# yzang2019/tendermint-fork

Hardware: AMD Instinct MI355X
Metric: ed25519 verifies/sec at 1/8 MI355X (higher is better)
Workload: dtype u32 (GF(2^255-19) radix 2^25.5 limbs, int64 accumulate); 1 GPU; C2: raw batch of 1048576 ed25519 signatures per GPU; signatures_per_gpu=1048576, key_cache=False, parallelism=shard-per-gpu x1

## Files before the change

### include/tmed25519.h

```cpp
#ifndef TMED25519_H
#define TMED25519_H

#include <stddef.h>
#include <stdint.h>

#ifdef __cplusplus
extern "C" {
#endif

#define TMED_OK 0
#define TMED_EINVAL (-1)
#define TMED_ENODEV (-2)
#define TMED_EHIP (-3)
#define TMED_ENOMEM (-4)
#define TMED_ENOKEYSET (-5)
#define TMED_EINTERNAL (-6)

typedef struct tmed_ctx tmed_ctx;

int tmed_device_count(void);

int tmed_init(int device, tmed_ctx **out);
void tmed_destroy(tmed_ctx *ctx);
const char *tmed_strerror(int code);

int tmed_verify_batch(tmed_ctx *ctx, const uint8_t *pubkeys, const uint8_t *sigs, const uint32_t *sig_lens,
                      const uint8_t *msgs, const uint32_t *msg_off, size_t n, uint8_t *out_valid);

int tmed_verify_batch_device(tmed_ctx *ctx, const uint8_t *d_pubkeys, const uint8_t *d_sigs,
                             const uint8_t *d_msgs, const uint32_t *d_msg_off, size_t n, uint8_t *d_out_valid,
                             void *stream);

int tmed_sign_batch(tmed_ctx *ctx, const uint8_t *seeds, const uint8_t *msgs, const uint32_t *msg_off, size_t n,
                    uint8_t *sigs_out, uint8_t *pubkeys_out);
int tmed_sign_batch_device(tmed_ctx *ctx, const uint8_t *d_seeds, const uint8_t *d_msgs, const uint32_t *d_msg_off,
                           size_t n, uint8_t *d_sigs_out, uint8_t *d_pubkeys_out, void *stream);

int tmed_window_stats(tmed_ctx *ctx, uint32_t lane_hist[65], uint32_t wave_hist[65]);

int tmed_b_window_bits(const tmed_ctx *ctx);
int tmed_keyset_b_window_bits(const tmed_ctx *ctx);
int tmed_keyset_a_window_bits(tmed_ctx *ctx, uint64_t handle);
int tmed_keyset_comb_entry(tmed_ctx *ctx, uint64_t handle, uint32_t key, int radix_bits, uint32_t window, uint32_t j,
                           int32_t out[30]);

float tmed_last_kernel_ms(tmed_ctx *ctx);

int tmed_set_kernel_timing(tmed_ctx *ctx, int on);
int tmed_kernel_times(tmed_ctx *ctx, float ms[3], int launches[3]);



int tmed_keyset_load(tmed_ctx *ctx, const uint8_t *pubkeys, size_t n, uint64_t *handle);
int tmed_keyset_free(tmed_ctx *ctx, uint64_t handle);
int tmed_keyset_extend(tmed_ctx *ctx, uint64_t handle, const uint8_t *pubkeys, size_t n, uint32_t *first_index);
int tmed_verify_batch_keyset(tmed_ctx *ctx, uint64_t handle, const uint32_t *val_idx, const uint8_t *sigs,
                             const uint32_t *sig_lens, const uint8_t *msgs, const uint32_t *msg_off, size_t n,
                             uint8_t *out_valid);
int tmed_verify_batch_keyset_device(tmed_ctx *ctx, uint64_t handle, const uint32_t *d_val_idx, const uint8_t *d_sigs,
                                    const uint8_t *d_msgs, const uint32_t *d_msg_off, size_t n, uint8_t *d_out_valid,
                                    void *stream);


int tmed_verify_batch_zip215(tmed_ctx *ctx, const uint8_t *pubkeys, const uint8_t *sigs, const uint32_t *sig_lens,
// ... 287 lines not shown
```

### tendermint-fork_amd/csrc/ctx.h

```cpp
#pragma once
#include <hip/hip_runtime.h>

#include <mutex>
#include <unordered_map>
#include <vector>

#include "../../include/tmed25519.h"
#include "kernels.h"
#include "keycache.h"

struct tmed_ctx;
struct BsStream;

namespace tmed {

struct DevBuf {
  void *p = nullptr;
  size_t cap = 0;
  hipError_t ensure(size_t bytes) {
    if (bytes <= cap) return hipSuccess;
    if (p) (void)hipFree(p);
    p = nullptr;
    cap = 0;
    size_t want = bytes + bytes / 4 + 256;
// ... 161 lines not shown
  int device = 0;
  hipStream_t stream = nullptr;
  hipStream_t copy_stream = nullptr;
  hipEvent_t ev0 = nullptr, ev1 = nullptr;
  float last_ms = 0.f;
  float last_copy_ms = 0.f, last_copy_gap_ms = 0.f;
  hipEvent_t trace_t0 = nullptr;
  float last_at[4] = {0, 0, 0, 0};
  std::mutex mu;
  int4 *d_bcomb = nullptr;
  int4 *d_b16 = nullptr;
  int4 *d_bcomb16 = nullptr;
  int4 *d_b26 = nullptr;
  int4 *d_b24 = nullptr;
  bool b24_tried = false;
  bool b24_on = true;
  bool acomb_on = true;
  int test_fail_ks_alloc = 0;
  int4 *d_slab = nullptr;
  int4 *d_prep = nullptr;
  int4 *d_fin = nullptr;
  int4 *d_fin_pre = nullptr;
  uint32_t slab_slots = 0;
  uint32_t chunk = 0;
  int main_waves = 6;
  uint32_t lat_max = 24576;
  int4 *d_glat = nullptr;
  uint32_t glat_max = 24576;
  bool timing = false;
  uint32_t last_hs_count = 0;
  tmed::KernelTimer timer;
  tmed::DevBuf d_a, d_b, d_msg, d_off, d_out, d_c;
  tmed::HostBuf h_a, h_b, h_msg, h_off, h_out, h_c;
  tmed::VoteSlot vslot[3];
  BsStream *bs = nullptr;
  tmed::Lane lane1;
  tmed::DevBuf d_merkle_lv, d_merkle_tab;
  std::vector<uint64_t> merkle_off;
  tmed::DevBuf d_proof_off, d_proof_out, d_proof_in;
  tmed::HostBuf h_csig;
  tmed::DevBuf d_csig;
  tmed::HostBuf h_hdr;
  tmed::DevBuf d_hdr;
  tmed::HostBuf h_med;
  tmed::DevBuf d_med;
  tmed::DevBuf d_korder;
// ... 19 lines not shown
  hipError_t e = hipSuccess;
  if (s == c->stream) {
    if (c->scratch_foreign) e = hipStreamWaitEvent(s, c->scratch_ev, 0);
  } else {
    if (!c->scratch_foreign) e = hipEventRecord(c->scratch_ev, c->stream);
    if (e == hipSuccess) e = hipStreamWaitEvent(s, c->scratch_ev, 0);
  }
  return e;
}
inline uint32_t last_chunk_count(uint32_t n, uint32_t chunk) {
  if (n == 0) return 0;
  const uint32_t m = n - (n - 1) / kFinCap * kFinCap;
  return m - (m - 1) / chunk * chunk;
}
inline bool generic_uses_glat(const tmed_ctx *c, uint32_t n) { return n <= c->glat_max; }
inline hipError_t generic_verify(tmed_ctx *c, const uint8_t *pub, const uint8_t *sig, const uint8_t *msgs,
                                 const uint32_t *off, uint32_t n, uint8_t *out, hipStream_t s, bool msg_slots,
                                 KernelTimer *timer, const VoteAsm *va = nullptr) {
  if (generic_uses_glat(c, n)) {
    c->last_hs_count = 0;
    return launch_verify_glat(pub, sig, msgs, off, n, out, c->d_bcomb16, c->d_glat, s, msg_slots, timer, va);
  }
  if (va) return hipErrorInvalidValue;
  hipError_t e = launch_verify(pub, sig, msgs, off, n, out, c->d_slab, c->slab_slots, BTabs{c->d_b16, c->d_bcomb16, c->d_b26},
                               c->d_prep, c->d_fin, c->d_fin_pre, s, c->chunk, c->main_waves, msg_slots, timer);
  c->last_hs_count = (e != hipSuccess || c->main_waves == 5) ? 0 : last_chunk_count(n, c->chunk);
  return e;
}
inline hipError_t scratch_release(tmed_ctx *c, hipStream_t s) {
  c->scratch_foreign = s != c->stream;
  return c->scratch_foreign ? hipEventRecord(c->scratch_ev, s) : hipSuccess;
}
}
```

### tendermint-fork_amd/csrc/kernels.h

```cpp
#pragma once
#include <hip/hip_runtime.h>
#include <stddef.h>
#include <stdint.h>

#include "ge25519.h"
#include "signbytes.h"

namespace tmed {

struct KernelTimer {
  static constexpr int kMax = 160;
  hipEvent_t ev[kMax];
  int kind[kMax];
  int n = 0;
  void mark(hipStream_t s, int k) {
    if (n < kMax) { kind[n] = k; (void)hipEventRecord(ev[n++], s); }
  }
};

constexpr uint32_t kThreadsPerBlock = 256;
constexpr uint32_t kSlabSlotBytes = 8 * 128;
constexpr uint32_t kSlabJointSlotBytes = 12 * 128;
inline size_t slab_bytes(uint32_t slots) { return (size_t)slots * kSlabJointSlotBytes; }

constexpr uint32_t kFinCap = 1u << 20;
constexpr int kFinInt4 = 8;
constexpr uint32_t kFinGroupMax = 16;
constexpr uint32_t kFinPreStride = kFinCap + 64;
constexpr size_t kFinBytes = (size_t)kFinCap * kFinInt4 * 16;
constexpr size_t kFinPreBytes = (size_t)kFinPreStride * 3 * 16;

struct BTabs {
  const int4 *b16;
  const int4 *comb16;
  const int4 *b26 = nullptr;
};
constexpr uint32_t kB26Entries = (1u << 25) + 1;
constexpr size_t kB26Bytes = 2 * (size_t)kB26Entries * 128;
hipError_t launch_build_b26(const int4 *comb16, int4 *tab, hipStream_t stream);
constexpr int kB24Windows = 11;
constexpr uint32_t kB24Entries = (1u << 23) + 1;
constexpr size_t kB24Bytes = (size_t)kB24Windows * kB24Entries * 128;
hipError_t launch_build_b24(const int4 *comb16, int4 *tab, hipStream_t stream);
constexpr uint32_t kB16Entries = 32769;
constexpr size_t kB16Bytes = (size_t)kB16Entries * 128;
hipError_t launch_build_b16(int4 *tab, hipStream_t stream);
constexpr size_t kBComb16Bytes = 16 * kB16Bytes;
void host_bcomb16_bases(int32_t out[16 * 40]);
hipError_t launch_build_bcomb16(const int32_t *d_bases, int4 *comb, hipStream_t stream);

hipError_t launch_verify(const uint8_t *pub, const uint8_t *sig, const uint8_t *msgs, const uint32_t *off,
                         uint32_t n, uint8_t *out, int4 *slab, uint32_t slab_stride, BTabs btab,
                         int4 *prep, int4 *fin, int4 *fin_pre, hipStream_t stream, uint32_t chunk = 0,
                         int main_waves = 6, bool msg_slots = false, KernelTimer *timer = nullptr,
                         bool zip215 = false);

hipError_t launch_verify_prep(const uint8_t *pub, const uint8_t *sig, const uint8_t *msgs, const uint32_t *off,
                              bool msg_slots, uint32_t base, uint32_t count, int4 *prep, uint32_t stride,
                              hipStream_t stream);
constexpr uint32_t kZipMax = 1u << 20;

hipError_t launch_sign(const uint8_t *seeds, const uint8_t *msgs, const uint32_t *off, uint32_t n, uint8_t *sig_out,
                       uint8_t *pub_out, const int4 *bcomb, hipStream_t stream);

constexpr uint32_t kPrepSlotBytes = 416;
constexpr uint32_t kPrepTailBytes = 256;

constexpr int kCombWindows = 32;
constexpr int kCombEntries = 129;
constexpr int kCombEntryInt4 = 8;
constexpr size_t kCombBytesPerKey = (size_t)kCombWindows * kCombEntries * kCombEntryInt4 * 16;
constexpr int kKeyChunkBits = 9;
constexpr uint32_t kKeyChunkKeys = 1u << kKeyChunkBits;
constexpr uint32_t kKeyChunksMax = (1u << 24) >> kKeyChunkBits;

// ... 63 lines not shown
```

### tendermint-fork_amd/csrc/kernels.hip

```cpp
#include "kernels.h"
#include "verify_core.h"
#include "verify_hs.h"
#include "kernel_util.h"
#include "rows.h"
#include "votes_dev.h"

namespace tmed {

__device__ int4 kIdentityRow[8] = {{1, 0, 0, 0}, {0, 0, 0, 0}, {1, 0, 0, 0}, {0, 0, 0, 0},
                                          {1, 0, 0, 0}, {0, 0, 0, 0}, {0, 0, 0, 0}, {0, 0, 0, 0}};

__device__ __forceinline__ void slab_st(int4 *p, int4 v) { *p = v; }
__device__ __forceinline__ int4 slab_ld(const int4 *p) { return *p; }

template <int ROWS>
struct SlabTabN {
  int4 *base;
  uint32_t slot;

  __device__ __forceinline__ const int4 *row(int j) const {
    return j == 0 ? kIdentityRow : base + ((size_t)slot * ROWS + (j - 1)) * 8;
  }

  __device__ __forceinline__ void store(int j, const ge_cached &c) const {
    if (j == 0) return;
    int4 *r = base + ((size_t)slot * ROWS + (j - 1)) * 8;
// ... 33 lines not shown

template <int BITS>
struct BPf {
  static constexpr int kBits = BITS;
  const int4 *tab;
  int4 *buf;
  uint32_t lane;
  __device__ __forceinline__ void prefetch(int j) const {
    __builtin_amdgcn_s_waitcnt(0xc07f);
#pragma unroll
    for (int q = 0; q < 8; q++)
      __builtin_amdgcn_global_load_lds((global_void *)(tab + (size_t)j * 8 + q), (lds_void *)(buf + q * 64), 16, 0, 0);
  }
  __device__ __forceinline__ void take(ge_niels &e) const { niels_load(e, buf + lane, 64); }
};

constexpr uint32_t kHsBlock = kThreadsPerBlock;

constexpr int kPrepWaves = 3;
__global__ __launch_bounds__(kHsBlock, kPrepWaves) void verify_prep_kernel(
    const uint8_t *__restrict__ pub, const uint8_t *__restrict__ sig, MsgSrc ms, uint32_t base, uint32_t count,
    int4 *__restrict__ prep, uint32_t stride, uint32_t *__restrict__ place) {
  const uint32_t slot = blockIdx.x * blockDim.x + threadIdx.x;
  if (place && slot == 0) place[0] = place[1] = 0;
  if (slot >= count) return;
  const uint32_t i = base + slot;
  uint32_t pw[8];
  bool sok;
  {
    uint32_t sw[16], k[8], h[16];
    load_row_words(pw, pub + 32 * (size_t)i, 2);
    load_row_words(sw, sig + 64 * (size_t)i, 4);
    const uint8_t *m;
    uint32_t mlen;
    ms.get(i, m, mlen);
    sok = (sw[15] & 0xE0000000u) == 0 && sc_is_canonical(sw + 8);
    sha512_stream(h, sw, pw, 64, m, mlen);
    sc_reduce512(k, h);
#pragma unroll
    for (int q = 0; q < 2; q++)
      prep[(size_t)q * stride + slot] = make_int4((int)k[4 * q], (int)k[4 * q + 1], (int)k[4 * q + 2], (int)k[4 * q + 3]);
#pragma unroll
    for (int q = 0; q < 2; q++) {
      const uint32_t *S = sw + 8 + 4 * q;
      prep[(size_t)(2 + q) * stride + slot] = sok ? make_int4((int)S[0], (int)S[1], (int)S[2], (int)S[3])
                                                  : make_int4(0, 0, 0, 0);
    }
// ... 113 lines not shown
  const int leader = __builtin_ctzll(act);
  fs = (uint32_t)__shfl((int)fs, leader);
  fl = (uint32_t)__shfl((int)fl, leader);
  const uint32_t pos = front ? fs + (uint32_t)__builtin_popcountll(sm & below)
                             : count - 1u - (fl + (uint32_t)__builtin_popcountll(act & ~sm & below));
#pragma unroll
  for (int q = 0; q < kPrepHsInt4; q++)
    prep2[(size_t)q * stride + pos] = make_int4(w[4 * q], w[4 * q + 1], w[4 * q + 2], w[4 * q + 3]);
}

struct HsDigitsDev {
  const int4 *p2;
  uint32_t stride, slot;
  bool active;
  __device__ __forceinline__ uint32_t word(int w) const {
    return active ? reinterpret_cast<const uint32_t *>(p2 + (size_t)(w >> 2) * stride + slot)[w & 3] : 0x88888888u;
  }
  __device__ __forceinline__ uint32_t cword(int w) const { return word(w); }
  __device__ __forceinline__ uint32_t dword(int w) const { return w < 5 ? word(8 + w) : 0x88888888u; }
};

constexpr int kHsWaves = 2;
template <int BB>
__global__ __launch_bounds__(kHsBlock, kHsWaves) void verify_main_hs_kernel(
    uint32_t base, uint32_t count, const int4 *__restrict__ prep, const int4 *__restrict__ prep2, uint32_t stride,
    int4 *__restrict__ slab, const int4 *__restrict__ btab, uint8_t *__restrict__ out, int zip215) {
  __shared__ int4 sbl[kHsBlock / 64][8 * 64];
  __shared__ int4 sbh[kHsBlock / 64][8 * 64];
  const uint32_t slot = blockIdx.x * blockDim.x + threadIdx.x;
  const bool active = slot < count;
  int32_t w[64];
#pragma unroll
  for (int q = 3; q < kPrepHsInt4; q++) {
    const int4 v = active ? prep2[(size_t)q * stride + slot] : make_int4(0, 0, 0, 0);
    w[4 * q] = v.x; w[4 * q + 1] = v.y; w[4 * q + 2] = v.z; w[4 * q + 3] = v.w;
  }
  uint32_t er[8];
#pragma unroll
  for (int j = 0; j < 8; j++) er[j] = (uint32_t)w[13 + j];
  if (BB == 16) {
    uint32_t e[8];
#pragma unroll
    for (int j = 0; j < 8; j++) e[j] = er[j];
    sc_recode_b<16>(er, e);
  }
  fe Rx, Ry;
#pragma unroll
  for (int j = 0; j < 10; j++) { Rx.v[j] = w[21 + j]; Ry.v[j] = w[31 + j]; }
  ge_p3 A;
#pragma unroll
  for (int j = 0; j < 10; j++) { A.X.v[j] = w[44 + j]; A.Y.v[j] = w[54 + j]; }
  if (!active) { fe_1(A.Y); fe_1(Ry); }
  fe_1(A.Z);
  fe_mul(A.T, A.X, A.Y);
  const int flags = w[41];
  int W = active ? (flags >> 8) : 29;
#pragma unroll
  for (int o = 32; o > 0; o >>= 1) {
    const int x = __shfl_xor(W, o);
    W = x > W ? x : W;
  }
  W = __builtin_amdgcn_readfirstlane(W);
  if (W < 29) W = 29;
  if (W > 64) W = 64;
  const uint32_t lane = threadIdx.x & 63u, wv = threadIdx.x >> 6;
  const HsDigitsDev ds{prep2, stride, slot, active};
  SlabTabJ tj{slab, slot};
  const size_t hi = BB == 26 ? (size_t)kB26Entries * kCombEntryInt4 : (size_t)8 * kB16Entries * kCombEntryInt4;
  BPf<BB> bl{btab, sbl[wv], lane};
  BPf<BB> bh{btab + hi, sbh[wv], lane};
  const bool id = verify_main_hsj(ds, (flags & 2) != 0, er, W, A, Rx, Ry, tj, bl, bh, zip215 != 0);
  if (active) out[base + (uint32_t)w[42]] = ((flags & 1) && id) ? 1 : 0;
}

__global__ __launch_bounds__(kThreadsPerBlock) void window_stats_kernel(const int4 *__restrict__ prep2, uint32_t stride,
                                                                       uint32_t count, uint32_t *__restrict__ lane_hist,
                                                                       uint32_t *__restrict__ wave_hist) {
  __shared__ uint32_t lh[65], wh[65];
  for (uint32_t b = threadIdx.x; b < 65; b += blockDim.x) lh[b] = wh[b] = 0;
  __syncthreads();
  const uint32_t slot = blockIdx.x * blockDim.x + threadIdx.x;
  const bool active = slot < count;
  int W = active ? (prep2[(size_t)10 * stride + slot].y >> 8) : 0;
  if (W < 0 || W > 64) W = 64;
  if (active) atomicAdd(&lh[W], 1u);
  int m = W;
#pragma unroll
  for (int o = 32; o > 0; o >>= 1) {
    const int x = __shfl_xor(m, o);
    m = x > m ? x : m;
  }
  if ((threadIdx.x & 63u) == 0 && slot < count) atomicAdd(&wh[m], 1u);
  __syncthreads();
  for (uint32_t b = threadIdx.x; b < 65; b += blockDim.x) {
    if (lh[b]) atomicAdd(&lane_hist[b], lh[b]);
// ... 105 lines not shown
__global__ __launch_bounds__(kThreadsPerBlock) void verify_finish_kernel(
    const int4 *__restrict__ fin, int4 *__restrict__ pre, const uint8_t *__restrict__ sig, uint8_t *__restrict__ out,
    uint32_t fin_base, uint32_t L, uint32_t m, const uint32_t *__restrict__ perm) {
  const uint32_t lane = blockIdx.x * blockDim.x + threadIdx.x;
  if (lane >= L) return;
  FinDev a{fin, pre, sig, out, fin_base, lane, L, m, perm};
  finish_group(a);
}

hipError_t launch_finish(const int4 *fin, int4 *pre, const uint8_t *sig, uint8_t *out, uint32_t fin_base, uint32_t m,
                         hipStream_t stream, const uint32_t *perm = nullptr) {
  if (m == 0) return hipSuccess;
  constexpr uint32_t kLanes = 65536;
  uint32_t G = (m + kLanes - 1) / kLanes;
  if (G < 1) G = 1;
  if (G > kFinGroupMax) G = kFinGroupMax;
  const uint32_t L = (m + G - 1) / G;
  hipLaunchKernelGGL(verify_finish_kernel, dim3((L + kThreadsPerBlock - 1) / kThreadsPerBlock),
                     dim3(kThreadsPerBlock), 0, stream, fin, pre, sig, out, fin_base, L, m, perm);
  return hipGetLastError();
}

hipError_t launch_verify(const uint8_t *pub, const uint8_t *sig, const uint8_t *msgs, const uint32_t *off,
                         uint32_t n, uint8_t *out, int4 *slab, uint32_t slab_stride, BTabs btab,
                         int4 *prep, int4 *fin, int4 *fin_pre, hipStream_t stream, uint32_t chunk, int main_waves,
                         bool msg_slots, KernelTimer *timer, bool zip215) {
  const MsgSrc ms{msgs, off, msg_slots};
  if (chunk == 0 || chunk > slab_stride) chunk = slab_stride;
  if (chunk % kThreadsPerBlock != 0 || slab_stride % kThreadsPerBlock != 0) return hipErrorInvalidValue;
  const bool hs = main_waves != 5 || zip215;
  uint32_t *place = reinterpret_cast<uint32_t *>(reinterpret_cast<char *>(prep) + (size_t)slab_stride * kPrepSlotBytes);
  if (timer) timer->mark(stream, -1);
  for (uint32_t fbase = 0; fbase < n; fbase += kFinCap) {
    const uint32_t m = (n - fbase) < kFinCap ? (n - fbase) : kFinCap;
    for (uint32_t base = fbase; base < fbase + m; base += chunk) {
      const uint32_t count = (fbase + m - base) < chunk ? (fbase + m - base) : chunk;
      const uint32_t blocks = (count + kThreadsPerBlock - 1) / kThreadsPerBlock;
      const uint32_t hblocks = (count + kHsBlock - 1) / kHsBlock;

      hipLaunchKernelGGL(verify_prep_kernel, dim3(hblocks), dim3(kHsBlock), 0, stream, pub, sig, ms, base,
                         count, prep, slab_stride, hs ? place : nullptr);
      if (timer) timer->mark(stream, 0);
      if (hs) {
        int4 *prep2 = prep + (size_t)kPrepInt4 * slab_stride;
        hipLaunchKernelGGL(verify_prep_r_kernel, dim3(hblocks), dim3(kHsBlock), 0, stream, sig, base, count,
                           prep, prep2, slab_stride, place, zip215 ? 1 : 0);
        if (timer) timer->mark(stream, 0);
        if (btab.b26)
          hipLaunchKernelGGL(verify_main_hs_kernel<26>, dim3(hblocks), dim3(kHsBlock), 0, stream, base, count,
                             prep, prep2, slab_stride, slab, btab.b26, out, zip215 ? 1 : 0);
        else
          hipLaunchKernelGGL(verify_main_hs_kernel<16>, dim3(hblocks), dim3(kHsBlock), 0, stream, base, count,
                             prep, prep2, slab_stride, slab, btab.comb16, out, zip215 ? 1 : 0);
      } else {
        hipLaunchKernelGGL(verify_main_kernel, dim3(blocks), dim3(kThreadsPerBlock), 0, stream, base, count, prep,
                           slab_stride, slab, btab.b16, fin, fbase, out);
      }
      if (timer) timer->mark(stream, 1);
      hipError_t e = hipGetLastError();
      if (e != hipSuccess) return e;
    }
    hipError_t e = hs ? hipSuccess : launch_finish(fin, fin_pre, sig, out, fbase, m, stream);
    if (timer) timer->mark(stream, 2);
    if (e != hipSuccess) return e;
  }
  return hipSuccess;
}

hipError_t launch_verify_prep(const uint8_t *pub, const uint8_t *sig, const uint8_t *msgs, const uint32_t *off,
                              bool msg_slots, uint32_t base, uint32_t count, int4 *prep, uint32_t stride,
                              hipStream_t stream) {
  if (count == 0) return hipSuccess;
  if (count > stride) return hipErrorInvalidValue;
  const MsgSrc ms{msgs, off, msg_slots};
  hipLaunchKernelGGL(verify_prep_kernel, dim3((count + kHsBlock - 1) / kHsBlock),
                     dim3(kHsBlock), 0, stream, pub, sig, ms, base, count, prep, stride, nullptr);
// ... 576 lines not shown
```

### tendermint-fork_amd/csrc/tmed_capi.hip

```cpp
#include <hip/hip_runtime.h>
#include <stdlib.h>
#include <string.h>

#include <algorithm>
#include <map>
#include <mutex>
#include <new>
#include <string>

#include "../../include/tmed25519.h"
#include "kernels.h"

#include "ctx.h"
#include "median_host.h"

using namespace tmed;

extern "C" {

int tmed_device_count(void) {
  int n = 0;
  if (hipGetDeviceCount(&n) != hipSuccess) return 0;
  return n;
}
// ... 97 lines not shown
  if (hipSetDevice(device) != hipSuccess) return TMED_EHIP;
  tmed_ctx *c = new tmed_ctx();
  c->device = device;
  hipError_t e = hipStreamCreateWithFlags(&c->stream, hipStreamNonBlocking);
  if (e == hipSuccess) e = hipStreamCreateWithFlags(&c->copy_stream, hipStreamNonBlocking);
  if (e == hipSuccess) e = hipEventCreate(&c->ev0);
  if (e == hipSuccess) e = hipEventCreate(&c->ev1);
  if (e == hipSuccess) e = hipEventCreateWithFlags(&c->scratch_ev, hipEventDisableTiming);
  auto round_up = [](uint32_t v) {
    if (v < kThreadsPerBlock) v = kThreadsPerBlock;
    if (v > (1u << 24)) v = 1u << 24;
    return (v + kThreadsPerBlock - 1) / kThreadsPerBlock * kThreadsPerBlock;
  };
  c->slab_slots = 4096 * kThreadsPerBlock;
  c->chunk = c->slab_slots;
  if (const char *v = getenv("TMED_SLAB_SLOTS")) c->slab_slots = round_up((uint32_t)strtoul(v, nullptr, 10));
  c->chunk = c->slab_slots;
  if (const char *v = getenv("TMED_CHUNK")) c->chunk = std::min(c->slab_slots, round_up((uint32_t)strtoul(v, nullptr, 10)));
  if (const char *v = getenv("TMED_MAIN_WAVES")) c->main_waves = atoi(v) == 5 ? 5 : 6;
  if (const char *v = getenv("TMED_LAT_MAX")) c->lat_max = (uint32_t)strtoul(v, nullptr, 10);
  if (c->lat_max > kLatMax) c->lat_max = kLatMax;
  if (const char *v = getenv("TMED_GLAT_MAX")) c->glat_max = (uint32_t)strtoul(v, nullptr, 10);
  if (c->glat_max > kGLatMax) c->glat_max = kGLatMax;
  if (e == hipSuccess)
    e = hipMalloc((void **)&c->d_slab, slab_bytes(c->slab_slots));
  if (e == hipSuccess) e = hipMalloc((void **)&c->d_prep, (size_t)c->slab_slots * kPrepSlotBytes + kPrepTailBytes);
  if (e == hipSuccess) e = hipMalloc((void **)&c->d_fin, kFinBytes);
  if (e == hipSuccess) e = hipMalloc((void **)&c->d_fin_pre, kFinPreBytes);
  if (e == hipSuccess) e = hipMalloc((void **)&c->d_glat, kGLatHandBytes);
  uint8_t *d_bpub = nullptr, *d_bok = nullptr;
  const uint8_t benc[32] = {0x58, 0x66, 0x66, 0x66, 0x66, 0x66, 0x66, 0x66, 0x66, 0x66, 0x66,
                            0x66, 0x66, 0x66, 0x66, 0x66, 0x66, 0x66, 0x66, 0x66, 0x66, 0x66,
                            0x66, 0x66, 0x66, 0x66, 0x66, 0x66, 0x66, 0x66, 0x66, 0x66};
  if (e == hipSuccess) e = hipMalloc((void **)&c->d_b16, kB16Bytes);
  if (e == hipSuccess) e = launch_build_b16(c->d_b16, c->stream);
  if (e == hipSuccess) e = hipMalloc((void **)&c->d_bcomb16, kBComb16Bytes);
  {
    static int32_t bases[16 * 40];
    static std::once_flag bases_once;
    std::call_once(bases_once, [] { host_bcomb16_bases(bases); });
    int32_t *d_bases = nullptr;
    if (e == hipSuccess) e = hipMalloc((void **)&d_bases, sizeof(bases));
    if (e == hipSuccess) e = hipMemcpy(d_bases, bases, sizeof(bases), hipMemcpyHostToDevice);
    if (e == hipSuccess) e = launch_build_bcomb16(d_bases, c->d_bcomb16, c->stream);
    if (e == hipSuccess) e = hipStreamSynchronize(c->stream);
    if (d_bases) (void)hipFree(d_bases);
  }
  if (e == hipSuccess && !env_off("TMED_B26")) c->d_b26 = bshare_acquire(0, device, c->d_bcomb16, c->stream);
  c->b24_on = !env_off("TMED_B24");
  c->acomb_on = !env_off("TMED_KS_ACOMB");
  if (const char *v = getenv("TMED_TEST_FAIL_KS_ALLOC")) c->test_fail_ks_alloc = atoi(v);
  c->kc_on = !env_off("TMED_KEYCACHE");
  if (const char *v = getenv("TMED_KEYCACHE_GB")) c->kc_budget = (size_t)strtoull(v, nullptr, 10) << 30;
  if (e == hipSuccess) e = hipMalloc((void **)&c->d_bcomb, kCombBytesPerKey);
  if (e == hipSuccess) e = hipMalloc((void **)&d_bpub, 32);
  if (e == hipSuccess) e = hipMalloc((void **)&d_bok, 1);
  if (e == hipSuccess) e = hipMemcpy(d_bpub, benc, 32, hipMemcpyHostToDevice);
  int rc = map_err(e);
  if (rc == TMED_OK) rc = build_comb(c, d_bpub, 1, 0, d_bok, c->d_bcomb);
  if (d_bpub) (void)hipFree(d_bpub);
  if (d_bok) (void)hipFree(d_bok);
  if (rc != TMED_OK) {
    tmed_destroy(c);
    return rc;
  }
  *out = c;
  return TMED_OK;
}

void tmed_destroy(tmed_ctx *c) {
  if (!c) return;
// ... 143 lines not shown
    if (!g_pinned.erase((uintptr_t)p)) return TMED_EINVAL;
  }
  return hipHostFree(p) == hipSuccess ? TMED_OK : TMED_EHIP;
}

int tmed_host_register(void *p, size_t bytes) {
  if (!p || bytes == 0) return TMED_EINVAL;
  if (hipHostRegister(p, bytes, hipHostRegisterDefault) != hipSuccess) return TMED_EHIP;
  std::lock_guard<std::mutex> lk(g_pin_mu);
  g_pinned[(uintptr_t)p] = (uintptr_t)p + bytes;
  return TMED_OK;
}

int tmed_host_unregister(void *p) {
  {
    std::lock_guard<std::mutex> lk(g_pin_mu);
    if (!p || !g_pinned.erase((uintptr_t)p)) return TMED_EINVAL;
  }
  return hipHostUnregister(p) == hipSuccess ? TMED_OK : TMED_EHIP;
}

int tmed_b_window_bits(const tmed_ctx *c) { return c && c->d_b26 ? 26 : 16; }
int tmed_keyset_b_window_bits(const tmed_ctx *c) { return c && c->d_b24 ? 24 : 16; }
int tmed_keyset_a_window_bits(tmed_ctx *c, uint64_t handle) {
  if (!c) return -1;
  std::lock_guard<std::mutex> lk(c->mu);
  const Keyset *k = find_keyset(c, handle);
  if (!k) return -1;
  return !k->comba.empty() && k->comba_n == k->n && c->d_b24 ? kCombABits : 8;
}

int tmed_keyset_comb_entry(tmed_ctx *c, uint64_t handle, uint32_t key, int radix_bits, uint32_t window, uint32_t j,
                           int32_t out[30]) {
  if (!c || !out) return TMED_EINVAL;
  std::lock_guard<std::mutex> lk(c->mu);
  const Keyset *k = find_keyset(c, handle);
  if (!k || key >= k->n) return TMED_EINVAL;
  const int4 *src;
  if (radix_bits == 8) {
    if (window >= (uint32_t)kCombWindows || j >= kCombEntries) return TMED_EINVAL;
    src = k->comb_row(key, (size_t)window * kCombEntries + j);
  } else if (radix_bits == kCombABits) {
    if (k->comba.empty() || key >= k->comba_n || window >= (uint32_t)kCombAWindows) return TMED_EINVAL;
    if (j >= (window + 1 == (uint32_t)kCombAWindows ? kCombATopEntries : kCombAEntries)) return TMED_EINVAL;
    src = k->comba_row_of(key, comba_row((int)window, j));
  } else {
// ... 154 lines not shown
```

### tendermint-fork_amd/csrc/zip215.hip

```cpp
#include <hip/hip_runtime.h>
#include <string.h>
#include <sys/random.h>

#include <stdio.h>
#include <stdlib.h>

#include <vector>

#include "ctx.h"
#include "kernel_util.h"
#include "verify_core.h"
#include "verify_hs.h"
#include "quad.h"

namespace tmed {

constexpr int kZipWin = 16;
constexpr int kZipZWin = 8;
constexpr uint32_t kZipRow = 8;
constexpr uint32_t kZipItemsMax = 16385;
__host__ __device__ __forceinline__ int zip_glog(int w) { return w < 8 ? 1 : (w < 15 ? 2 : 0); }
__host__ __device__ __forceinline__ uint32_t zip_groups(int w) { return w < 8 ? 16385u : (w < 15 ? 8193u : 4098u); }
__host__ __device__ __forceinline__ uint32_t zip_h(int w) { return w == 15 ? 2u : 1u; }
__host__ __device__ __forceinline__ uint32_t zip_level_items(int w, int level) {
// ... 729 lines not shown
  if (e != hipSuccess) return map_err(e);
  memset(g_zip_stats, 0, sizeof g_zip_stats);
  const uint32_t chunk = std::min<uint32_t>(kZipMax, c->slab_slots);
  for (uint32_t base = 0; base < n; base += chunk) {
    const uint32_t N = n - base < chunk ? n - base : chunk;
    uint8_t seed[32];
    if (g_zip_fixed) memcpy(seed, g_zip_seed, 32);
    else if (getrandom(seed, 32, 0) != 32) return TMED_EHIP;
    e = hipMemcpyAsync(z.seed, seed, 32, hipMemcpyHostToDevice, s);
    if (e != hipSuccess) return map_err(e);
    g_zip_stats[0]++;
    constexpr uint32_t kZipSinglyMin = 1u << 14;
    if (N >= kZipSinglyMin && c->zip_count_pending) {
      e = hipEventSynchronize(c->zip_ev);
      if (e != hipSuccess) return map_err(e);
      c->zip_count_pending = false;
      c->zip_dense = *static_cast<const uint32_t *>(c->h_zip.p) != 0;
    }
    if (c->zip_dense && N >= kZipSinglyMin) {
      g_zip_stats[2]++;
      g_zip_stats[3] += N;
      const uint8_t *gm = msg_slots ? msgs + (size_t)base * kVoteSlot : msgs;
      e = launch_verify(pub + 32 * (size_t)base, sig + 64 * (size_t)base, gm, off + base, N, out + base, c->d_slab,
                        c->slab_slots, BTabs{c->d_b16, c->d_bcomb16, c->d_b26}, c->d_prep, c->d_fin, c->d_fin_pre, s,
                        c->chunk, 6, msg_slots, nullptr, true);
      if (e == hipSuccess && !c->zip_ev) e = hipEventCreateWithFlags(&c->zip_ev, hipEventDisableTiming);
      if (e == hipSuccess) e = c->h_zip.ensure(4);
      if (e == hipSuccess) e = hipMemsetAsync(z.flag, 0, 4, s);
      if (e == hipSuccess)
        hipLaunchKernelGGL(zip_count_fail_kernel, dim3((N + 4095) / 4096), dim3(256), 0, s, out + base, N, z.flag);
      if (e == hipSuccess) e = hipGetLastError();
      if (e == hipSuccess) e = hipMemcpyAsync(c->h_zip.p, z.flag, 4, hipMemcpyDeviceToHost, s);
      if (e == hipSuccess) e = hipEventRecord(c->zip_ev, s);
      if (e != hipSuccess) return map_err(e);
      c->zip_count_pending = true;
      continue;
    }
    const uint32_t blocks = (N + kThreadsPerBlock - 1) / kThreadsPerBlock;
    e = launch_verify_prep(pub, sig, msgs, off, msg_slots, base, N, c->d_prep, c->slab_slots, s);
    if (e != hipSuccess) return map_err(e);
    hipLaunchKernelGGL(zip_prep_r_kernel, dim3(blocks), dim3(kThreadsPerBlock), 0, s, sig, base, N, c->d_prep,
                       c->slab_slots, z.seed, (uint64_t)base, z.pts, z.dig, z.cs, kZipMax, out);
    constexpr uint32_t kZipMinGroup = 1u << 14;
    std::vector<std::pair<uint32_t, uint32_t>> level{{0u, N}}, single;
    while (!level.empty()) {
      std::vector<std::pair<uint32_t, uint32_t>> failed;
      for (auto &g : level) {
// ... 5 lines not shown
        g_zip_stats[1]++;
        if (!ok) failed.push_back(g);
      }
      const bool dense = level.size() >= 2 && failed.size() * 2 > level.size();
      std::vector<std::pair<uint32_t, uint32_t>> next;
      for (auto &g : failed) {
        if (!dense && g.second >= 2 * kZipMinGroup) {
          const uint32_t h = g.second / 2;
          next.push_back({g.first, h});
          next.push_back({g.first + h, g.second - h});
        } else {
          single.push_back(g);
        }
      }
      level.swap(next);
    }
    if (N >= kZipSinglyMin) c->zip_dense = !single.empty();
    for (auto &g : single) {
      g_zip_stats[2]++;
      g_zip_stats[3] += g.second;
      const uint32_t lo = base + g.first;
      const uint8_t *gm = msg_slots ? msgs + (size_t)lo * kVoteSlot : msgs;
      e = launch_verify(pub + 32 * (size_t)lo, sig + 64 * (size_t)lo, gm, off + lo, g.second, out + lo, c->d_slab,
                        c->slab_slots, BTabs{c->d_b16, c->d_bcomb16, c->d_b26}, c->d_prep, c->d_fin, c->d_fin_pre, s, c->chunk,
                        6, msg_slots, nullptr, true);
      if (e != hipSuccess) return map_err(e);
    }
  }
  c->last_hs_count = 0;
  return TMED_OK;
}

}

extern "C" {

int tmed_zip215_set_seed(const uint8_t *seed32) {
  const char *t = getenv("TMED_ZIP215_TEST_SEED");
  if (seed32 && !(t && t[0] == '1')) return TMED_EINVAL;
  if (seed32) {
    memcpy(g_zip_seed, seed32, 32);
    g_zip_fixed = true;
  } else {
    g_zip_fixed = false;
  }
  return TMED_OK;
}
// ... 62 lines not shown
```

### tendermint-fork_amd/tmed/_native.py

```python
from __future__ import annotations

import ctypes
import os

PKG_ROOT = os.path.dirname(os.path.dirname(os.path.abspath(__file__)))
LIB_PATH = os.environ.get("TMED_LIB") or os.path.join(PKG_ROOT, "lib", "libtmed25519_hip.so")

TMED_OK = 0
TMED_EINVAL = -1
TMED_ENODEV = -2
TMED_EHIP = -3
TMED_ENOMEM = -4
TMED_ENOKEYSET = -5
TMED_EINTERNAL = -6

_lib = None


class TmedError(RuntimeError):
    def __init__(self, code: int, what: str = ""):
        self.code = code
        msg = lib().tmed_strerror(code).decode() if _lib is not None else str(code)
        super().__init__("%s: %s (code %d)" % (what or "tmed", msg, code))

# ... 39 lines not shown
    l.tmed_keycache_stats.argtypes = [P, P]
    l.tmed_keycache_wait.restype = I
    l.tmed_keycache_wait.argtypes = [P]
    l.tmed_keycache_flush.restype = I
    l.tmed_keycache_flush.argtypes = [P]
    l.tmed_keycache_warm.restype = I
    l.tmed_keycache_warm.argtypes = [P, P]
    l.tmed_verify_batch_keyset.restype = I
    l.tmed_verify_batch_keyset.argtypes = [P, ctypes.c_uint64, P, P, P, P, P, SZ, P]
    l.tmed_verify_batch_keyset_device.restype = I
    l.tmed_verify_batch_keyset_device.argtypes = [P, ctypes.c_uint64, P, P, P, P, SZ, P, P]
    l.tmed_set_kernel_timing.restype = I
    l.tmed_set_kernel_timing.argtypes = [P, I]
    l.tmed_kernel_times.restype = I
    l.tmed_kernel_times.argtypes = [P, ctypes.POINTER(ctypes.c_float), ctypes.POINTER(ctypes.c_int)]
    l.tmed_last_kernel_ms.restype = ctypes.c_float
    l.tmed_last_kernel_ms.argtypes = [P]
    l.tmed_window_stats.restype = I
    l.tmed_window_stats.argtypes = [P, P, P]
    l.tmed_b_window_bits.restype = I
    l.tmed_b_window_bits.argtypes = [P]
    l.tmed_keyset_b_window_bits.restype = I
    l.tmed_keyset_b_window_bits.argtypes = [P]
    l.tmed_keyset_a_window_bits.restype = I
    l.tmed_keyset_a_window_bits.argtypes = [P, ctypes.c_uint64]
    l.tmed_keyset_comb_entry.restype = I
    l.tmed_keyset_comb_entry.argtypes = [P, ctypes.c_uint64, ctypes.c_uint32, ctypes.c_int, ctypes.c_uint32,
                                         ctypes.c_uint32, P]
    l.tmed_host_alloc.restype = I
    l.tmed_host_alloc.argtypes = [SZ, ctypes.POINTER(ctypes.c_void_p)]
    l.tmed_host_free.restype = I
    l.tmed_host_free.argtypes = [P]
    l.tmed_host_register.restype = I
    l.tmed_host_register.argtypes = [P, SZ]
    l.tmed_host_unregister.restype = I
    l.tmed_host_unregister.argtypes = [P]
    l.tmed_verify_batch_zip215.argtypes = [P, P, P, P, P, P, SZ, P]
    l.tmed_verify_batch_zip215_device.argtypes = [P, P, P, P, P, SZ, P, P]
    l.tmed_zip215_set_seed.argtypes = [P]
    l.tmed_zip215_stats.argtypes = [P]
    l.tmed_test_pool_jitter.restype = None
    l.tmed_test_pool_jitter.argtypes = [I]
    l.tmed_test_stream_delay.restype = None
    l.tmed_test_stream_delay.argtypes = [I]
    l.tmed_test_joint_rows.restype = I
    l.tmed_test_joint_rows.argtypes = [P, P, P, P, SZ, P]
    l.tmed_debug_zero_bits.restype = I
    l.tmed_debug_zero_bits.argtypes = [P, SZ, ctypes.POINTER(SZ)]
    _lib = l
    return l


EXPORTED_SYMBOLS = [
    "tmed_device_count", "tmed_init", "tmed_destroy", "tmed_strerror",
    "tmed_verify_batch", "tmed_verify_batch_device",
    "tmed_sign_batch", "tmed_sign_batch_device", "tmed_last_kernel_ms",
    "tmed_vote_sign_bytes", "tmed_valu_peak", "tmed_verify_commits", "tmed_verify_commits_with",
    "tmed_test_pool_jitter", "tmed_test_stream_delay", "tmed_test_joint_rows", "tmed_debug_zero_bits",
    "tmed_keyset_load", "tmed_keyset_free", "tmed_keyset_extend", "tmed_verify_batch_keyset",
    "tmed_keycache_config", "tmed_keycache_stats", "tmed_keycache_flush", "tmed_keycache_warm", "tmed_keycache_wait", "tmed_verify_batch_keyset_device",
    "tmed_set_kernel_timing", "tmed_kernel_times", "tmed_blocksync_verify", "tmed_blocksync_submit", "tmed_blocksync_wait",
    "tmed_merkle_roots", "tmed_valset_hashes", "tmed_header_hashes", "tmed_partset_roots",
    "tmed_commit_hashes", "tmed_txs_hashes",
    "tmed_merkle_proofs", "tmed_partset_proofs", "tmed_txs_proofs", "tmed_merkle_proofs_verify",
    "tmed_light_verify", "tmed_light_verify_with",
    "tmed_median_times", "tmed_median_times_host",
    "tmed_verify_commits_multi", "tmed_blocksync_verify_multi", "tmed_window_stats", "tmed_b_window_bits", "tmed_keyset_b_window_bits", "tmed_keyset_a_window_bits", "tmed_keyset_comb_entry", "tmed_seam_phase_us",
    "tmed_verify_batch_zip215", "tmed_verify_batch_zip215_device", "tmed_zip215_set_seed", "tmed_zip215_stats",
    "tmed_host_alloc", "tmed_host_free", "tmed_host_register", "tmed_host_unregister",
]
```

### tendermint-fork_amd/tmed/engine.py

```python
from __future__ import annotations

import ctypes
from typing import Sequence

import numpy as np

from ._native import TMED_OK, TmedError, lib


def _p(a: np.ndarray):
    return a.ctypes.data_as(ctypes.c_void_p)


def pack_messages(msgs: Sequence[bytes]):
    lens = np.fromiter((len(m) for m in msgs), dtype=np.int64, count=len(msgs))
    off = np.zeros(len(msgs) + 1, dtype=np.int64)
    np.cumsum(lens, out=off[1:])
    if off[-1] >= 2**32:
        raise ValueError("message batch exceeds 4 GiB")
    flat = np.frombuffer(b"".join(msgs), dtype=np.uint8) if off[-1] else np.zeros(1, np.uint8)
    return flat, off.astype(np.uint32)


class PinnedBuffer:
# ... 224 lines not shown

    def set_kernel_timing(self, on: bool) -> None:
        rc = lib().tmed_set_kernel_timing(self._h, 1 if on else 0)
        if rc != TMED_OK:
            raise TmedError(rc, "tmed_set_kernel_timing")

    def kernel_times(self):
        ms, n = (ctypes.c_float * 3)(), (ctypes.c_int * 3)()
        rc = lib().tmed_kernel_times(self._h, ms, n)
        if rc != TMED_OK:
            raise TmedError(rc, "tmed_kernel_times")
        return list(ms), list(n)

    def window_stats(self):
        lh, wh = np.zeros(65, np.uint32), np.zeros(65, np.uint32)
        rc = lib().tmed_window_stats(self._h, _p(lh), _p(wh))
        if rc != TMED_OK:
            raise TmedError(rc, "tmed_window_stats")
        return lh, wh

    def b_window_bits(self) -> int:
        return int(lib().tmed_b_window_bits(self._h))

    def keyset_b_window_bits(self) -> int:
        return int(lib().tmed_keyset_b_window_bits(self._h))

    def keyset_a_window_bits(self, handle: int) -> int:
        return int(lib().tmed_keyset_a_window_bits(self._h, handle))

    def keyset_comb_entry(self, handle: int, key: int, radix_bits: int, window: int, j: int) -> np.ndarray:
        out = np.zeros(30, np.int32)
        rc = lib().tmed_keyset_comb_entry(self._h, handle, key, radix_bits, window, j, out.ctypes.data)
        if rc != 0:
            raise TmedError(rc, "tmed_keyset_comb_entry")
        return out

    def last_kernel_ms(self) -> float:
        return float(lib().tmed_last_kernel_ms(self._h))
```

Measured before the change: 107.4 million verifies/s.

## Make HS main verify kernel persistent with per-wave atomic group claiming

The main HS verify kernel becomes a persistent grid, sized to the resident block count from the occupancy API. Each wave atomically claims 64-signature groups until the work runs out. The per-lane slab scratch is now indexed by resident thread slot rather than signature slot, so the slab allocation shrinks to resident lanes only. This is meant to reduce tail imbalance from variable window counts and to shrink the slab's memory footprint, which may improve cache locality. It adds one atomic per group and depends on the occupancy query being accurate.

```diff
diff --git a/include/tmed25519.h b/include/tmed25519.h
--- a/include/tmed25519.h
+++ b/include/tmed25519.h
@@ -40,6 +40,7 @@
 
 int tmed_b_window_bits(const tmed_ctx *ctx);
 int tmed_keyset_b_window_bits(const tmed_ctx *ctx);
+int tmed_main_resident_lanes(const tmed_ctx *ctx);
 int tmed_keyset_a_window_bits(tmed_ctx *ctx, uint64_t handle);
 int tmed_keyset_comb_entry(tmed_ctx *ctx, uint64_t handle, uint32_t key, int radix_bits, uint32_t window, uint32_t j,
                            int32_t out[30]);
diff --git a/tendermint-fork_amd/csrc/ctx.h b/tendermint-fork_amd/csrc/ctx.h
--- a/tendermint-fork_amd/csrc/ctx.h
+++ b/tendermint-fork_amd/csrc/ctx.h
@@ -207,6 +207,7 @@
   int4 *d_fin = nullptr;
   int4 *d_fin_pre = nullptr;
   uint32_t slab_slots = 0;
+  uint32_t hs_blocks = 0;
   uint32_t chunk = 0;
   int main_waves = 6;
   uint32_t lat_max = 24576;
@@ -272,7 +273,8 @@
     return launch_verify_glat(pub, sig, msgs, off, n, out, c->d_bcomb16, c->d_glat, s, msg_slots, timer, va);
   }
   if (va) return hipErrorInvalidValue;
-  hipError_t e = launch_verify(pub, sig, msgs, off, n, out, c->d_slab, c->slab_slots, BTabs{c->d_b16, c->d_bcomb16, c->d_b26},
+  hipError_t e = launch_verify(pub, sig, msgs, off, n, out, c->d_slab, c->slab_slots, c->hs_blocks,
+                               BTabs{c->d_b16, c->d_bcomb16, c->d_b26},
                                c->d_prep, c->d_fin, c->d_fin_pre, s, c->chunk, c->main_waves, msg_slots, timer);
   c->last_hs_count = (e != hipSuccess || c->main_waves == 5) ? 0 : last_chunk_count(n, c->chunk);
   return e;
diff --git a/tendermint-fork_amd/csrc/kernels.h b/tendermint-fork_amd/csrc/kernels.h
--- a/tendermint-fork_amd/csrc/kernels.h
+++ b/tendermint-fork_amd/csrc/kernels.h
@@ -21,7 +21,12 @@
 constexpr uint32_t kThreadsPerBlock = 256;
 constexpr uint32_t kSlabSlotBytes = 8 * 128;
 constexpr uint32_t kSlabJointSlotBytes = 12 * 128;
-inline size_t slab_bytes(uint32_t slots) { return (size_t)slots * kSlabJointSlotBytes; }
+inline size_t slab_hs_bytes(uint32_t hs_blocks) { return (size_t)hs_blocks * kThreadsPerBlock * kSlabJointSlotBytes; }
+inline size_t slab_bytes(uint32_t slots, uint32_t hs_blocks, int main_waves) {
+  const size_t hs = slab_hs_bytes(hs_blocks), full = (size_t)slots * kSlabSlotBytes;
+  return main_waves == 5 && full > hs ? full : hs;
+}
+hipError_t main_hs_resident_blocks(int device, bool b26, uint32_t *blocks);
 
 constexpr uint32_t kFinCap = 1u << 20;
 constexpr int kFinInt4 = 8;
@@ -50,7 +55,7 @@
 hipError_t launch_build_bcomb16(const int32_t *d_bases, int4 *comb, hipStream_t stream);
 
 hipError_t launch_verify(const uint8_t *pub, const uint8_t *sig, const uint8_t *msgs, const uint32_t *off,
-                         uint32_t n, uint8_t *out, int4 *slab, uint32_t slab_stride, BTabs btab,
+                         uint32_t n, uint8_t *out, int4 *slab, uint32_t slab_stride, uint32_t hs_blocks, BTabs btab,
                          int4 *prep, int4 *fin, int4 *fin_pre, hipStream_t stream, uint32_t chunk = 0,
                          int main_waves = 6, bool msg_slots = false, KernelTimer *timer = nullptr,
                          bool zip215 = false);
diff --git a/tendermint-fork_amd/csrc/kernels.hip b/tendermint-fork_amd/csrc/kernels.hip
--- a/tendermint-fork_amd/csrc/kernels.hip
+++ b/tendermint-fork_amd/csrc/kernels.hip
@@ -2,6 +2,7 @@
 #include "verify_core.h"
 #include "verify_hs.h"
 #include "kernel_util.h"
+#include "main_claim.h"
 #include "rows.h"
 #include "votes_dev.h"
 
@@ -81,7 +82,7 @@
     const uint8_t *__restrict__ pub, const uint8_t *__restrict__ sig, MsgSrc ms, uint32_t base, uint32_t count,
     int4 *__restrict__ prep, uint32_t stride, uint32_t *__restrict__ place) {
   const uint32_t slot = blockIdx.x * blockDim.x + threadIdx.x;
-  if (place && slot == 0) place[0] = place[1] = 0;
+  if (place && slot == 0) place[0] = place[1] = place[2] = 0;
   if (slot >= count) return;
   const uint32_t i = base + slot;
   uint32_t pw[8];
@@ -241,13 +242,10 @@
 
 constexpr int kHsWaves = 2;
 template <int BB>
-__global__ __launch_bounds__(kHsBlock, kHsWaves) void verify_main_hs_kernel(
-    uint32_t base, uint32_t count, const int4 *__restrict__ prep, const int4 *__restrict__ prep2, uint32_t stride,
-    int4 *__restrict__ slab, const int4 *__restrict__ btab, uint8_t *__restrict__ out, int zip215) {
-  __shared__ int4 sbl[kHsBlock / 64][8 * 64];
-  __shared__ int4 sbh[kHsBlock / 64][8 * 64];
-  const uint32_t slot = blockIdx.x * blockDim.x + threadIdx.x;
-  const bool active = slot < count;
+__device__ __forceinline__ void main_hs_group(uint32_t base, const int4 *__restrict__ prep2, uint32_t stride,
+                                              uint32_t slot, bool active, int4 *__restrict__ slab, uint32_t tslot,
+                                              const int4 *__restrict__ btab, int4 *sbl, int4 *sbh, uint32_t lane,
+                                              uint8_t *__restrict__ out, int zip215) {
   int32_t w[64];
 #pragma unroll
   for (int q = 3; q < kPrepHsInt4; q++) {
@@ -282,14 +280,49 @@
   W = __builtin_amdgcn_readfirstlane(W);
   if (W < 29) W = 29;
   if (W > 64) W = 64;
-  const uint32_t lane = threadIdx.x & 63u, wv = threadIdx.x >> 6;
   const HsDigitsDev ds{prep2, stride, slot, active};
-  SlabTabJ tj{slab, slot};
+  SlabTabJ tj{slab, tslot};
   const size_t hi = BB == 26 ? (size_t)kB26Entries * kCombEntryInt4 : (size_t)8 * kB16Entries * kCombEntryInt4;
-  BPf<BB> bl{btab, sbl[wv], lane};
-  BPf<BB> bh{btab + hi, sbh[wv], lane};
+  BPf<BB> bl{btab, sbl, lane};
+  BPf<BB> bh{btab + hi, sbh, lane};
   const bool id = verify_main_hsj(ds, (flags & 2) != 0, er, W, A, Rx, Ry, tj, bl, bh, zip215 != 0);
   if (active) out[base + (uint32_t)w[42]] = ((flags & 1) && id) ? 1 : 0;
+}
+
+template <int BB>
+__global__ __launch_bounds__(kHsBlock, kHsWaves) void verify_main_hs_kernel(
+    uint32_t base, uint32_t count, const int4 *__restrict__ prep, const int4 *__restrict__ prep2, uint32_t stride,
+    int4 *__restrict__ slab, const int4 *__restrict__ btab, uint8_t *__restrict__ out, int zip215,
+    uint32_t *__restrict__ claim) {
+  __shared__ int4 sbl[kHsBlock / 64][8 * 64];
+  __shared__ int4 sbh[kHsBlock / 64][8 * 64];
+  const uint32_t wv = (uint32_t)__builtin_amdgcn_readfirstlane((int)(threadIdx.x >> 6));
+#pragma unroll 1
+  for (;;) {
+    uint32_t z = 0;
+    asm volatile("" : "+v"(z));
+    const uint32_t lane = __builtin_amdgcn_mbcnt_hi(~0u, __builtin_amdgcn_mbcnt_lo(~0u, z));
+    const uint32_t tslot = (blockIdx.x * (kHsBlock / 64) + wv) * 64 + lane;
+    uint32_t g = 0;
+    if (lane == 0) g = atomicAdd(claim, 1u);
+    g = (uint32_t)__builtin_amdgcn_readfirstlane((int)g);
+    HsGroup grp;
+    if (!hs_claim_group(g, count, grp)) break;
+    main_hs_group<BB>(base, prep2, stride, grp.base + lane, lane < grp.nact, slab, tslot, btab, sbl[wv], sbh[wv], lane,
+                      out, zip215);
+  }
+}
+
+hipError_t main_hs_resident_blocks(int device, bool b26, uint32_t *blocks) {
+  int cus = 0, per_cu = 0;
+  hipError_t e = hipDeviceGetAttribute(&cus, hipDeviceAttributeMultiprocessorCount, device);
+  if (e == hipSuccess)
+    e = b26 ? hipOccupancyMaxActiveBlocksPerMultiprocessor(&per_cu, verify_main_hs_kernel<26>, (int)kHsBlock, 0)
+            : hipOccupancyMaxActiveBlocksPerMultiprocessor(&per_cu, verify_main_hs_kernel<16>, (int)kHsBlock, 0);
+  if (e != hipSuccess) return e;
+  if (cus <= 0 || per_cu <= 0) return hipErrorInvalidValue;
+  *blocks = (uint32_t)cus * (uint32_t)per_cu;
+  return hipSuccess;
 }
 
 __global__ __launch_bounds__(kThreadsPerBlock) void window_stats_kernel(const int4 *__restrict__ prep2, uint32_t stride,
@@ -441,13 +474,14 @@
 }
 
 hipError_t launch_verify(const uint8_t *pub, const uint8_t *sig, const uint8_t *msgs, const uint32_t *off,
-                         uint32_t n, uint8_t *out, int4 *slab, uint32_t slab_stride, BTabs btab,
+                         uint32_t n, uint8_t *out, int4 *slab, uint32_t slab_stride, uint32_t hs_blocks, BTabs btab,
                          int4 *prep, int4 *fin, int4 *fin_pre, hipStream_t stream, uint32_t chunk, int main_waves,
                          bool msg_slots, KernelTimer *timer, bool zip215) {
   const MsgSrc ms{msgs, off, msg_slots};
   if (chunk == 0 || chunk > slab_stride) chunk = slab_stride;
   if (chunk % kThreadsPerBlock != 0 || slab_stride % kThreadsPerBlock != 0) return hipErrorInvalidValue;
   const bool hs = main_waves != 5 || zip215;
+  if (hs && hs_blocks == 0) return hipErrorInvalidValue;
   uint32_t *place = reinterpret_cast<uint32_t *>(reinterpret_cast<char *>(prep) + (size_t)slab_stride * kPrepSlotBytes);
   if (timer) timer->mark(stream, -1);
   for (uint32_t fbase = 0; fbase < n; fbase += kFinCap) {
@@ -465,12 +499,13 @@
         hipLaunchKernelGGL(verify_prep_r_kernel, dim3(hblocks), dim3(kHsBlock), 0, stream, sig, base, count,
                            prep, prep2, slab_stride, place, zip215 ? 1 : 0);
         if (timer) timer->mark(stream, 0);
+        const uint32_t mblocks = hs_grid_blocks(count, hs_blocks, kHsBlock / 64);
         if (btab.b26)
-          hipLaunchKernelGGL(verify_main_hs_kernel<26>, dim3(hblocks), dim3(kHsBlock), 0, stream, base, count,
-                             prep, prep2, slab_stride, slab, btab.b26, out, zip215 ? 1 : 0);
+          hipLaunchKernelGGL(verify_main_hs_kernel<26>, dim3(mblocks), dim3(kHsBlock), 0, stream, base, count,
+                             prep, prep2, slab_stride, slab, btab.b26, out, zip215 ? 1 : 0, place + 2);
         else
-          hipLaunchKernelGGL(verify_main_hs_kernel<16>, dim3(hblocks), dim3(kHsBlock), 0, stream, base, count,
-                             prep, prep2, slab_stride, slab, btab.comb16, out, zip215 ? 1 : 0);
+          hipLaunchKernelGGL(verify_main_hs_kernel<16>, dim3(mblocks), dim3(kHsBlock), 0, stream, base, count,
+                             prep, prep2, slab_stride, slab, btab.comb16, out, zip215 ? 1 : 0, place + 2);
       } else {
         hipLaunchKernelGGL(verify_main_kernel, dim3(blocks), dim3(kThreadsPerBlock), 0, stream, base, count, prep,
                            slab_stride, slab, btab.b16, fin, fbase, out);
diff --git a/tendermint-fork_amd/csrc/main_claim.h b/tendermint-fork_amd/csrc/main_claim.h
--- /dev/null
+++ b/tendermint-fork_amd/csrc/main_claim.h
@@ -0,0 +1,37 @@
+#pragma once
+#include <stdint.h>
+
+#ifndef TMED_HD
+#if defined(__HIPCC__)
+#include <hip/hip_runtime.h>
+#define TMED_HD __host__ __device__ __forceinline__
+#else
+#define TMED_HD static inline
+#endif
+#endif
+
+namespace tmed {
+
+constexpr uint32_t kHsGroup = 64;
+
+TMED_HD uint32_t hs_group_count(uint32_t count) { return count / kHsGroup + (count % kHsGroup != 0 ? 1u : 0u); }
+
+struct HsGroup {
+  uint32_t base, nact;
+};
+TMED_HD bool hs_claim_group(uint32_t g, uint32_t count, HsGroup &r) {
+  if (g >= hs_group_count(count)) return false;
+  r.base = g * kHsGroup;
+  const uint32_t left = count - r.base;
+  r.nact = left < kHsGroup ? left : kHsGroup;
+  return true;
+}
+TMED_HD uint64_t hs_group_mask(const HsGroup &r) { return r.nact >= 64 ? ~0ull : (1ull << r.nact) - 1ull; }
+
+TMED_HD uint32_t hs_grid_blocks(uint32_t count, uint32_t resident_blocks, uint32_t waves_per_block) {
+  const uint32_t g = hs_group_count(count);
+  const uint32_t need = g / waves_per_block + (g % waves_per_block != 0 ? 1u : 0u);
+  return need < resident_blocks ? need : resident_blocks;
+}
+
+}
diff --git a/tendermint-fork_amd/csrc/tmed_capi.hip b/tendermint-fork_amd/csrc/tmed_capi.hip
--- a/tendermint-fork_amd/csrc/tmed_capi.hip
+++ b/tendermint-fork_amd/csrc/tmed_capi.hip
@@ -143,8 +143,6 @@
   if (c->lat_max > kLatMax) c->lat_max = kLatMax;
   if (const char *v = getenv("TMED_GLAT_MAX")) c->glat_max = (uint32_t)strtoul(v, nullptr, 10);
   if (c->glat_max > kGLatMax) c->glat_max = kGLatMax;
-  if (e == hipSuccess)
-    e = hipMalloc((void **)&c->d_slab, slab_bytes(c->slab_slots));
   if (e == hipSuccess) e = hipMalloc((void **)&c->d_prep, (size_t)c->slab_slots * kPrepSlotBytes + kPrepTailBytes);
   if (e == hipSuccess) e = hipMalloc((void **)&c->d_fin, kFinBytes);
   if (e == hipSuccess) e = hipMalloc((void **)&c->d_fin_pre, kFinPreBytes);
@@ -168,6 +166,8 @@
     if (d_bases) (void)hipFree(d_bases);
   }
   if (e == hipSuccess && !env_off("TMED_B26")) c->d_b26 = bshare_acquire(0, device, c->d_bcomb16, c->stream);
+  if (e == hipSuccess) e = main_hs_resident_blocks(device, c->d_b26 != nullptr, &c->hs_blocks);
+  if (e == hipSuccess) e = hipMalloc((void **)&c->d_slab, slab_bytes(c->slab_slots, c->hs_blocks, c->main_waves));
   c->b24_on = !env_off("TMED_B24");
   c->acomb_on = !env_off("TMED_KS_ACOMB");
   if (const char *v = getenv("TMED_TEST_FAIL_KS_ALLOC")) c->test_fail_ks_alloc = atoi(v);
@@ -357,6 +357,7 @@
 
 int tmed_b_window_bits(const tmed_ctx *c) { return c && c->d_b26 ? 26 : 16; }
 int tmed_keyset_b_window_bits(const tmed_ctx *c) { return c && c->d_b24 ? 24 : 16; }
+int tmed_main_resident_lanes(const tmed_ctx *c) { return c ? (int)(c->hs_blocks * kThreadsPerBlock) : 0; }
 int tmed_keyset_a_window_bits(tmed_ctx *c, uint64_t handle) {
   if (!c) return -1;
   std::lock_guard<std::mutex> lk(c->mu);
diff --git a/tendermint-fork_amd/csrc/zip215.hip b/tendermint-fork_amd/csrc/zip215.hip
--- a/tendermint-fork_amd/csrc/zip215.hip
+++ b/tendermint-fork_amd/csrc/zip215.hip
@@ -775,7 +775,7 @@
       g_zip_stats[3] += N;
       const uint8_t *gm = msg_slots ? msgs + (size_t)base * kVoteSlot : msgs;
       e = launch_verify(pub + 32 * (size_t)base, sig + 64 * (size_t)base, gm, off + base, N, out + base, c->d_slab,
-                        c->slab_slots, BTabs{c->d_b16, c->d_bcomb16, c->d_b26}, c->d_prep, c->d_fin, c->d_fin_pre, s,
+                        c->slab_slots, c->hs_blocks, BTabs{c->d_b16, c->d_bcomb16, c->d_b26}, c->d_prep, c->d_fin, c->d_fin_pre, s,
                         c->chunk, 6, msg_slots, nullptr, true);
       if (e == hipSuccess && !c->zip_ev) e = hipEventCreateWithFlags(&c->zip_ev, hipEventDisableTiming);
       if (e == hipSuccess) e = c->h_zip.ensure(4);
@@ -827,7 +827,7 @@
       const uint32_t lo = base + g.first;
       const uint8_t *gm = msg_slots ? msgs + (size_t)lo * kVoteSlot : msgs;
       e = launch_verify(pub + 32 * (size_t)lo, sig + 64 * (size_t)lo, gm, off + lo, g.second, out + lo, c->d_slab,
-                        c->slab_slots, BTabs{c->d_b16, c->d_bcomb16, c->d_b26}, c->d_prep, c->d_fin, c->d_fin_pre, s, c->chunk,
+                        c->slab_slots, c->hs_blocks, BTabs{c->d_b16, c->d_bcomb16, c->d_b26}, c->d_prep, c->d_fin, c->d_fin_pre, s, c->chunk,
                         6, msg_slots, nullptr, true);
       if (e != hipSuccess) return map_err(e);
     }
diff --git a/tendermint-fork_amd/tmed/_native.py b/tendermint-fork_amd/tmed/_native.py
--- a/tendermint-fork_amd/tmed/_native.py
+++ b/tendermint-fork_amd/tmed/_native.py
@@ -85,6 +85,8 @@
     l.tmed_b_window_bits.argtypes = [P]
     l.tmed_keyset_b_window_bits.restype = I
     l.tmed_keyset_b_window_bits.argtypes = [P]
+    l.tmed_main_resident_lanes.restype = I
+    l.tmed_main_resident_lanes.argtypes = [P]
     l.tmed_keyset_a_window_bits.restype = I
     l.tmed_keyset_a_window_bits.argtypes = [P, ctypes.c_uint64]
     l.tmed_keyset_comb_entry.restype = I
@@ -128,7 +130,7 @@
     "tmed_merkle_proofs", "tmed_partset_proofs", "tmed_txs_proofs", "tmed_merkle_proofs_verify",
     "tmed_light_verify", "tmed_light_verify_with",
     "tmed_median_times", "tmed_median_times_host",
-    "tmed_verify_commits_multi", "tmed_blocksync_verify_multi", "tmed_window_stats", "tmed_b_window_bits", "tmed_keyset_b_window_bits", "tmed_keyset_a_window_bits", "tmed_keyset_comb_entry", "tmed_seam_phase_us",
+    "tmed_verify_commits_multi", "tmed_blocksync_verify_multi", "tmed_window_stats", "tmed_b_window_bits", "tmed_keyset_b_window_bits", "tmed_main_resident_lanes", "tmed_keyset_a_window_bits", "tmed_keyset_comb_entry", "tmed_seam_phase_us",
     "tmed_verify_batch_zip215", "tmed_verify_batch_zip215_device", "tmed_zip215_set_seed", "tmed_zip215_stats",
     "tmed_host_alloc", "tmed_host_free", "tmed_host_register", "tmed_host_unregister",
 ]
diff --git a/tendermint-fork_amd/tmed/engine.py b/tendermint-fork_amd/tmed/engine.py
--- a/tendermint-fork_amd/tmed/engine.py
+++ b/tendermint-fork_amd/tmed/engine.py
@@ -270,6 +270,9 @@
     def b_window_bits(self) -> int:
         return int(lib().tmed_b_window_bits(self._h))
 
+    def main_resident_lanes(self) -> int:
+        return int(lib().tmed_main_resident_lanes(self._h))
+
     def keyset_b_window_bits(self) -> int:
         return int(lib().tmed_keyset_b_window_bits(self._h))
 
```

Result: no change. 106.4 million verifies/s (-0.9%).
